# CPestka/Tensor-FFT

Measured on AMD Instinct MI355X. Metric: Gsamples/s + %fp16-MFMA-peak, batched N=4096 fp16 C2C FFT, higher is better.
Workload: dtype f16

## Files before the change

tensor-fft_amd/conv/conv4096.hpp:

```cpp
#pragma once

#include "../csrc/k4096.hpp"

namespace conv4096 {

using k4096::f4;
using k4096::h8;
using k4096::s4;
using k4096::u2;
using k4096::u4;

__host__ __device__ constexpr uint32_t filter_slot(uint32_t k) {
  const uint32_t k0 = k & 15, k1 = (k >> 4) & 15, k2 = k >> 8;
  const uint32_t half = k0 >> 3, j = k0 & 7, g = k2 >> 2, r2 = k2 & 3;
  return ((half * 4 + r2) * 64 + 16 * g + k1) * 8 + j;
}

__global__ __launch_bounds__(k4096::kThreads, 2) void conv4096_kernel(
    const uint16_t* in_re, const uint16_t* in_im, uint16_t* out_re, uint16_t* out_im, uint64_t in_stride, uint64_t out_stride,
    uint32_t batch, uint32_t live, uint32_t filters, const uint8_t* __restrict__ tables, const uint16_t* __restrict__ filt) {
  using namespace k4096;
  extern __shared__ __attribute__((aligned(16))) uint8_t lds[];
  const int tid = threadIdx.x;
  const int lane = tid & 63;
  const int wave = __builtin_amdgcn_readfirstlane(tid >> 6);

  uint8_t* const wl = lds + kLdsTableBytes + wave * kLdsWaveBytes;
  const uint32_t wl_off = __builtin_amdgcn_readfirstlane(
      static_cast<uint32_t>(reinterpret_cast<uintptr_t>((__attribute__((address_space(3))) uint8_t*)wl)));

  const uint32_t stride_b = gridDim.x * live;
  uint32_t b = static_cast<uint32_t>(wave) < live ? blockIdx.x * live + wave : batch;

  for (int i = tid; i < kLdsTableBytes / 16; i += kThreads)
    reinterpret_cast<u4*>(lds)[i] = reinterpret_cast<const u4*>(tables + kOffG)[i];

  const h8 f_re = *reinterpret_cast<const h8*>(tables + kOffF1 + lane * 32);
  const h8 f_im = *reinterpret_cast<const h8*>(tables + kOffF1 + lane * 32 + 16);
  const f4 tw_re = *reinterpret_cast<const f4*>(tables + kOffTw + lane * 32);
  const f4 tw_im = *reinterpret_cast<const f4*>(tables + kOffTw + lane * 32 + 16);
  asm volatile("s_waitcnt vmcnt(0)" ::: "memory");
  __syncthreads();
  if (b >= batch) return;
  dma_in<true>(reinterpret_cast<const uint8_t*>(in_re + b * in_stride), reinterpret_cast<const uint8_t*>(in_im + b * in_stride), wl_off, lane);

  const uint8_t* const g_tab = lds + lane * 16;
  const uint8_t* const h_tab = lds + 16384 + lane * 16;

  const int g = lane >> 4, q = (lane >> 2) & 3, p = lane & 3;
  const int m = q + 4 * (g & 1), bb = g >> 1;
  uint8_t* const tr_base = wl + m * 1024 + bb * 512 + 8 * p;

  auto transform = [&](auto&& mul, auto&& sink) {
    uint32_t pr[8][4], pi[8][4];
#pragma unroll
    for (int t = 0; t < 8; ++t) {
      f4 dre[2], dim[2];
#pragma unroll
      for (int e = 0; e < 2; ++e) {
        const int n1 = 2 * t + e;
        uint8_t* a = tr_base + 32 * (n1 ^ m);
        const s4 xr = __builtin_amdgcn_ds_read_tr16_b64_v4i16((__attribute__((address_space(3))) s4*)(a));
        const s4 xi = __builtin_amdgcn_ds_read_tr16_b64_v4i16((__attribute__((address_space(3))) s4*)(a + 8192));
        const u4 raw = {__builtin_bit_cast(u2, xr).x, __builtin_bit_cast(u2, xr).y, __builtin_bit_cast(u2, xi).x, __builtin_bit_cast(u2, xi).y};
        const h8 x = __builtin_bit_cast(h8, raw);
        dre[e] = mfma(f_re, x);
        dim[e] = mfma(f_im, x);
      }
#pragma unroll
      for (int r = 0; r < 4; ++r) {
        pr[t][r] = pk(dre[0][r], dre[1][r]);
        pi[t][r] = pk(dim[0][r], dim[1][r]);
      }
    }
#pragma unroll
    for (int pp = 0; pp < 2; ++pp)
#pragma unroll
      for (int r = 0; r < 4; ++r) {
        transpose4(pr[0 + pp][r], pr[2 + pp][r], pr[4 + pp][r], pr[6 + pp][r]);
        transpose4(pi[0 + pp][r], pi[2 + pp][r], pi[4 + pp][r], pi[6 + pp][r]);
      }
    auto tile23 = [&](int k0, f4& o_re, f4& o_im) {
      const int a = k0 >> 2, r = k0 & 3;
      const u4 araw = {pr[2 * a][r], pr[2 * a + 1][r], pi[2 * a][r], pi[2 * a + 1][r]};
      const h8 aop = __builtin_bit_cast(h8, araw);
      const u4 graw = *reinterpret_cast<const u4*>(g_tab + k0 * 1024);
      const f4 e_re = mfma(aop, __builtin_bit_cast(h8, graw));
      const f4 e_im = mfma(aop, im_form(graw));
      f4 t_re, t_im;
#pragma unroll
      for (int r4 = 0; r4 < 4; ++r4) {
        t_re[r4] = __builtin_fmaf(e_re[r4], tw_re[r4], -(e_im[r4] * tw_im[r4]));
        t_im[r4] = __builtin_fmaf(e_re[r4], tw_im[r4], e_im[r4] * tw_re[r4]);
      }
      const u4 braw = {pk(t_re[0], t_re[1]), pk(t_re[2], t_re[3]), pk(t_im[0], t_im[1]), pk(t_im[2], t_im[3])};
      const h8 bop = __builtin_bit_cast(h8, braw);
      const u4 hraw = *reinterpret_cast<const u4*>(h_tab + k0 * 1024);
      o_re = mfma(__builtin_bit_cast(h8, hraw), bop);
      o_im = mfma(im_form(hraw), bop);
      mul(k0, o_re, o_im);
    };
#pragma unroll
    for (int half = 0; half < 2; ++half) {
      uint32_t ore[4][4], oim[4][4];
#pragma unroll
      for (int kp = 0; kp < 4; ++kp) {
        f4 e_re, e_im, o_re, o_im;
        tile23(8 * half + 2 * kp, e_re, e_im);
        tile23(8 * half + 2 * kp + 1, o_re, o_im);
#pragma unroll
        for (int r2 = 0; r2 < 4; ++r2) {
          ore[r2][kp] = pk(e_re[r2], o_re[r2]);
          oim[r2][kp] = pk(e_im[r2], o_im[r2]);
        }
      }
#pragma unroll
      for (int r2 = 0; r2 < 4; ++r2) {
        const u4 vr = {ore[r2][0], ore[r2][1], ore[r2][2], ore[r2][3]};
        const u4 vi = {oim[r2][0], oim[r2][1], oim[r2][2], oim[r2][3]};
        sink(half, r2, vr, vi);
      }
    }
  };

  for (;;) {
    asm volatile("s_waitcnt vmcnt(0)" ::: "memory");

    const uint16_t* const fimg = filt + static_cast<uint64_t>(b % filters) * 8192u + 8u * lane;
    u4 hre[2][4], him[2][4];
#pragma unroll
    for (int half = 0; half < 2; ++half)
#pragma unroll
      for (int r2 = 0; r2 < 4; ++r2) {
        hre[half][r2] = *reinterpret_cast<const u4*>(fimg + (half * 4 + r2) * 512);
        him[half][r2] = *reinterpret_cast<const u4*>(fimg + 4096 + (half * 4 + r2) * 512);
      }

    transform(
        [&](int k0, f4& o_re, f4& o_im) {
#pragma unroll
          for (int r2 = 0; r2 < 4; ++r2) {
            const float fr = static_cast<float>(__builtin_bit_cast(h8, hre[k0 >> 3][r2])[k0 & 7]) * 4096.f;
            const float fi = static_cast<float>(__builtin_bit_cast(h8, him[k0 >> 3][r2])[k0 & 7]) * 4096.f;
            const float zr = __builtin_fmaf(o_re[r2], fr, -(o_im[r2] * fi));
            o_im[r2] = __builtin_fmaf(o_re[r2], fi, o_im[r2] * fr);
            o_re[r2] = zr;
          }
        },
        [&](int half, int r2, u4 vr, u4 vi) {
          const uint32_t mm = 2u * g + (r2 >> 1);
          const uint32_t cl = 2u * (lane & 15) + half + 32u * (r2 & 1);
          const uint32_t off = 1024u * mm + 16u * (cl ^ (2u * mm));
          *reinterpret_cast<u4*>(wl + 8192 + off) = vr;
          *reinterpret_cast<u4*>(wl + off) = vi;
        });
    asm volatile("s_waitcnt lgkmcnt(0)" ::: "memory");

    transform([](int, f4&, f4&) {},
              [&](int half, int r2, u4 vr, u4 vi) {
                const uint32_t slot = 2u * (lane & 15) + half;
                const uint32_t off = 16u * (slot ^ ((slot >> 3) & 1)) + 512u * (4 * g + r2);
                *reinterpret_cast<u4*>(wl + 8192 + off) = vr;
                *reinterpret_cast<u4*>(wl + off) = vi;
              });
    uint16_t* const y_re = out_re + b * out_stride;
    uint16_t* const y_im = out_im + b * out_stride;
    const uint32_t rd = 16u * (lane ^ ((lane >> 3) & 1));
#pragma unroll
    for (int i = 0; i < 8; ++i) {
      const u4 vr = *reinterpret_cast<const u4*>(wl + 1024 * i + rd);
      const u4 vi = *reinterpret_cast<const u4*>(wl + 8192 + 1024 * i + rd);
      st<kNonTemporal>(y_re + 512 * i + 8 * lane, vr);
      st<kNonTemporal>(y_im + 512 * i + 8 * lane, vi);
    }
    const uint32_t nb = b + stride_b;
    if (nb >= batch) break;
    asm volatile("s_waitcnt lgkmcnt(0)" ::: "memory");
    dma_in<true>(reinterpret_cast<const uint8_t*>(in_re + nb * in_stride), reinterpret_cast<const uint8_t*>(in_im + nb * in_stride), wl_off, lane);
    b = nb;
  }
}

}
```

tensor-fft_amd/conv/tfft_conv.hip:

```cpp
#include <hip/hip_runtime.h>

#include <algorithm>
#include <cstring>
#include <mutex>
#include <string>
#include <vector>

#include "../../include/tfft_conv.h"
#include "cmul.hpp"
#include "conv4096.hpp"

namespace {

thread_local std::string g_err;

int fail(int code, const std::string& msg) {
  g_err = msg;
  return code;
}
int hip_fail(hipError_t e, const char* what) { return fail(TFFT_ERR_HIP, std::string(what) + ": " + hipGetErrorString(e)); }
int pass_through(int rc) {
  if (rc != TFFT_OK) g_err = tfft_last_error();
  return rc;
}
#define CONV_HIP(call)                        \
  do {                                        \
    const hipError_t e_ = (call);             \
    if (e_ != hipSuccess) return hip_fail(e_, #call); \
  } while (0)

inline bool is_pow2(uint64_t v) { return v && !(v & (v - 1)); }
inline int ilog2(uint64_t v) {
  int l = 0;
  while (v >>= 1) ++l;
  return l;
}

constexpr uint64_t kMinN = 256, kMaxN = uint64_t{1} << 26;

int check_abi() {
  static const int version = tfft_abi_version();
  if (version != TFFT_ABI_VERSION)
    return fail(TFFT_ERR_ARG, "libtfft.so speaks ABI " + std::to_string(version) + ", libtfft_conv.so was built against ABI " +
                                  std::to_string(TFFT_ABI_VERSION) + ": rebuild the add-on");
  return TFFT_OK;
}

int check_shape(uint64_t n, uint64_t batch, uint64_t filters, int flags) {
  if (!is_pow2(n)) return fail(TFFT_ERR_ARG, "n must be a power of two");
  if (n < kMinN || n > kMaxN) return fail(TFFT_ERR_ARG, "n must lie in 256 .. 2^26");
  if (flags & ~TFFT_CONV_COMPOSED) return fail(TFFT_ERR_ARG, "unknown flag bits (" + std::to_string(flags) + ")");
  if (batch == 0 || batch > 0xffffffffull) return fail(TFFT_ERR_ARG, "batch must be in [1, 2^32)");
  if (filters == 0 || filters > batch) return fail(TFFT_ERR_ARG, "filters must be in [1, batch]");
  return TFFT_OK;
}
int check_stride(uint64_t n, uint64_t stride, const char* which) {
  if (stride && (stride % 8 || stride < 2 * n))
    return fail(TFFT_ERR_ARG, std::string(which) + "_batch_stride must be 0 or a multiple of 8 that is >= 2 n");
  return TFFT_OK;
}

inline bool fused_shape(uint64_t n, int flags) { return n == 4096 && !(flags & TFFT_CONV_COMPOSED); }

uint64_t filter_slot(uint64_t n, int flags, uint64_t k) {
  if (fused_shape(n, flags)) return conv4096::filter_slot(static_cast<uint32_t>(k));
  const uint64_t n2 = tfft_plan_transposed_n2(n);
  if (!n2) return k;
  const uint64_t n1 = n / n2;
  return (k % n1) * n2 + k / n1;
}

bool planes_overlap(const void* pa, uint64_t sa, const void* pb, uint64_t sb, uint64_t batch, uint64_t n) {
  const uintptr_t a = reinterpret_cast<uintptr_t>(pa), b = reinterpret_cast<uintptr_t>(pb);
  const uintptr_t a_end = a + 2 * ((batch - 1) * sa + n), b_end = b + 2 * ((batch - 1) * sb + n);
  if (a_end <= b || b_end <= a) return false;
  if (batch == 1 || sa != sb) return true;
  const uint64_t d = static_cast<uint64_t>(a > b ? a - b : b - a) / 2 % sa;
  return d < n || sa - d < n;
}

inline size_t round256(size_t v) { return (v + 255) & ~size_t{255}; }

int describe_chain(uint64_t n, uint64_t batch, bool inverse, std::string& out) {
  char a[256], b[256];
  const uint64_t n2 = tfft_plan_transposed_n2(n);
  if (!n2) {
    const int rc = pass_through(tfft_plan_describe(n, 1, tfft_plan_default_variant(n, 1, batch), a, sizeof(a)));
    out = a;
    return rc;
  }
  const uint64_t n1 = n / n2;
  int rc = pass_through(tfft_plan_describe(n1, n2, n1 == 512 ? TFFT_VARIANT_RADIX512_ONE_PASS : 0, a, sizeof(a)));
  if (rc == TFFT_OK) rc = pass_through(tfft_plan_describe(n2, 1, 0, b, sizeof(b)));
  if (rc) return rc;
  out = inverse ? std::string(b) + " " + a : std::string(a) + " " + b;
  return TFFT_OK;
}

}

struct tfft_conv_plan {
  uint64_t n = 0, batch = 0, filters = 0, in_stride = 0, out_stride = 0;
  int device = 0, flags = 0, num_cus = 256;
  bool fused = false;
  void* d_tables = nullptr;
  uint16_t* d_filter = nullptr;
  bool have_filter = false;
  tfft_plan* fwd = nullptr;
  tfft_plan* inv = nullptr;
  size_t spec_bytes = 0, sub_bytes = 0;
  mutable std::mutex ws_mutex;
  mutable void* ws = nullptr;
  mutable size_t ws_bytes = 0;
  mutable bool ws_owned = false;
};

namespace {

int bind_workspace(const tfft_conv_plan* p) {
  if (!p->sub_bytes) return TFFT_OK;
  void* sub = static_cast<uint8_t*>(p->ws) + p->spec_bytes;
  int rc = pass_through(tfft_plan_set_workspace(p->fwd, tfft_plan_workspace_bytes(p->fwd) ? sub : nullptr, p->sub_bytes));
  if (rc == TFFT_OK) rc = pass_through(tfft_plan_set_workspace(p->inv, tfft_plan_workspace_bytes(p->inv) ? sub : nullptr, p->sub_bytes));
  return rc;
}

int ensure_workspace(const tfft_conv_plan* p) {
  std::lock_guard<std::mutex> lock(p->ws_mutex);
  const size_t need = p->spec_bytes + p->sub_bytes;
  if (!need || p->ws) return TFFT_OK;
  void* mem = nullptr;
  CONV_HIP(hipMalloc(&mem, need));
  p->ws = mem;
  p->ws_bytes = need;
  p->ws_owned = true;
  return bind_workspace(p);
}

void conv4096_shape(const tfft_conv_plan* p, uint32_t& live, uint32_t& grid) {
  const uint64_t cus = static_cast<uint64_t>(p->num_cus);
  live = 8;
  for (uint32_t l = 1; l <= 4; l *= 2)
    if (p->batch <= cus * l) {
      live = l;
      break;
    }
  const uint64_t blocks = (p->batch + live - 1) / live;
  const uint64_t iters = blocks >= 4 * cus ? 2 : 1;
  grid = static_cast<uint32_t>(std::max<uint64_t>(std::min<uint64_t>(blocks, cus), (blocks + iters - 1) / iters));
}

int create_fused(tfft_conv_plan* p) {
  std::vector<uint8_t> blob;
  k4096::build_tables(blob);
  CONV_HIP(hipMalloc(&p->d_tables, k4096::kOffF1n));
  CONV_HIP(hipMemcpy(p->d_tables, blob.data(), k4096::kOffF1n, hipMemcpyHostToDevice));
  CONV_HIP(hipFuncSetAttribute(reinterpret_cast<const void*>(conv4096::conv4096_kernel), hipFuncAttributeMaxDynamicSharedMemorySize, k4096::kLdsBytes));
  return TFFT_OK;
}

int create_composed(tfft_conv_plan* p) {
  const bool transposed = tfft_plan_transposed_n2(p->n) != 0;
  tfft_plan_opts fo = TFFT_PLAN_OPTS_INIT;
  fo.in_batch_stride = p->in_stride;
  fo.out_batch_stride = 2 * p->n;
  fo.preserve_input = 1;
  fo.output_order = transposed ? TFFT_ORDER_TRANSPOSED : TFFT_ORDER_NATURAL;
  tfft_plan_opts io = TFFT_PLAN_OPTS_INIT;
  io.in_batch_stride = 2 * p->n;
  io.out_batch_stride = p->out_stride;
  io.input_order = transposed ? TFFT_ORDER_TRANSPOSED : TFFT_ORDER_NATURAL;
  int rc = pass_through(tfft_plan_create(p->n, p->batch, p->device, &fo, &p->fwd));
  if (rc == TFFT_OK) rc = pass_through(tfft_plan_create(p->n, p->batch, p->device, &io, &p->inv));
  if (rc) return rc;
  p->spec_bytes = round256(static_cast<size_t>(p->batch) * p->n * 4);
  p->sub_bytes = round256(std::max(tfft_plan_workspace_bytes(p->fwd), tfft_plan_workspace_bytes(p->inv)));
  return TFFT_OK;
}

}

extern "C" {

const char* tfft_conv_last_error(void) { return g_err.c_str(); }

uint64_t tfft_conv_filter_slot(uint64_t n, int flags, uint64_t k) {
  if (!is_pow2(n) || n < kMinN || n > kMaxN || (flags & ~TFFT_CONV_COMPOSED) || k >= n) return UINT64_MAX;
  return filter_slot(n, flags, k);
}

int tfft_conv_describe(uint64_t n, uint64_t batch, uint64_t filters, int flags, char* buf, size_t bytes) {
  g_err.clear();
  if (!buf || bytes == 0) return fail(TFFT_ERR_ARG, "null buffer");
  int rc = check_shape(n, batch, filters, flags);
  if (rc) return rc;
  std::string out;
  if (fused_shape(n, flags)) {
    out = "conv4096:4096";
  } else {
    std::string f, i;
    rc = describe_chain(n, batch, false, f);
    if (rc == TFFT_OK) rc = describe_chain(n, batch, true, i);
    if (rc) return rc;
    out = f + " | cmul | " + i;
  }
  if (out.size() + 1 > bytes) return fail(TFFT_ERR_ARG, "buffer too small");
  std::memcpy(buf, out.c_str(), out.size() + 1);
  return TFFT_OK;
}

int tfft_conv_plan_create(uint64_t n, uint64_t batch, uint64_t filters, int device_id, uint64_t in_batch_stride,
                          uint64_t out_batch_stride, int flags, tfft_conv_plan** out) {
  g_err.clear();
  if (!out) return fail(TFFT_ERR_ARG, "null plan pointer");
  *out = nullptr;
  int rc = check_shape(n, batch, filters, flags);
  if (rc == TFFT_OK) rc = check_stride(n, in_batch_stride, "in");
  if (rc == TFFT_OK) rc = check_stride(n, out_batch_stride, "out");
  if (rc == TFFT_OK) rc = check_abi();
  if (rc == TFFT_OK) rc = pass_through(tfft_device_check(device_id));
  if (rc) return rc;
  int prev = 0;
  CONV_HIP(hipGetDevice(&prev));
  CONV_HIP(hipSetDevice(device_id));
  tfft_conv_plan* p = new tfft_conv_plan;
  p->n = n;
  p->batch = batch;
  p->filters = filters;
  p->in_stride = in_batch_stride ? in_batch_stride : 2 * n;
  p->out_stride = out_batch_stride ? out_batch_stride : 2 * n;
  p->device = device_id;
  p->flags = flags;
  p->fused = fused_shape(n, flags);
  hipDeviceProp_t prop;
  if (hipGetDeviceProperties(&prop, device_id) == hipSuccess) p->num_cus = prop.multiProcessorCount;
  rc = p->fused ? create_fused(p) : create_composed(p);
  if (rc == TFFT_OK) {
    const hipError_t e = hipMalloc(reinterpret_cast<void**>(&p->d_filter), static_cast<size_t>(filters) * n * 4);
    if (e != hipSuccess) rc = hip_fail(e, "hipMalloc(filter image)");
  }
  (void)hipSetDevice(prev);
  if (rc) {
    const std::string keep = g_err;
    tfft_conv_plan_destroy(p);
    g_err = keep;
    return rc;
  }
  *out = p;
  return TFFT_OK;
}

void tfft_conv_plan_destroy(tfft_conv_plan* p) {
  if (!p) return;
  tfft_plan_destroy(p->fwd);
  tfft_plan_destroy(p->inv);
  if (p->d_tables) (void)hipFree(p->d_tables);
  if (p->d_filter) (void)hipFree(p->d_filter);
  if (p->ws && p->ws_owned) (void)hipFree(p->ws);
  delete p;
}

int tfft_conv_plan_set_filter(tfft_conv_plan* p, const void* h_re, const void* h_im, void* stream) {
  g_err.clear();
  if (!p) return fail(TFFT_ERR_ARG, "null plan");
  if (!h_re || !h_im) return fail(TFFT_ERR_ARG, "null filter pointer");
  int cur = 0;
  CONV_HIP(hipGetDevice(&cur));
  if (cur != p->device) return fail(TFFT_ERR_ARG, "plan was created for another device than the current one");
  const size_t plane = static_cast<size_t>(p->filters) * p->n;
  std::vector<uint16_t> re(plane), im(plane), img(2 * plane);
  hipStream_t s = static_cast<hipStream_t>(stream);
  CONV_HIP(hipMemcpyAsync(re.data(), h_re, plane * 2, hipMemcpyDeviceToHost, s));
  CONV_HIP(hipMemcpyAsync(im.data(), h_im, plane * 2, hipMemcpyDeviceToHost, s));
  CONV_HIP(hipStreamSynchronize(s));
  for (uint64_t f = 0; f < p->filters; ++f)
    for (uint64_t k = 0; k < p->n; ++k) {
      const uint64_t slot = filter_slot(p->n, p->flags, k);
      img[f * 2 * p->n + slot] = re[f * p->n + k];
      img[f * 2 * p->n + p->n + slot] = im[f * p->n + k];
    }
  if (p->have_filter) CONV_HIP(hipDeviceSynchronize());
  CONV_HIP(hipMemcpy(p->d_filter, img.data(), img.size() * 2, hipMemcpyHostToDevice));
  p->have_filter = true;
  return TFFT_OK;
}

size_t tfft_conv_plan_workspace_bytes(const tfft_conv_plan* p) { return p ? p->spec_bytes + p->sub_bytes : 0; }

int tfft_conv_plan_set_workspace(tfft_conv_plan* p, void* device_ptr, size_t bytes) {
  g_err.clear();
  if (!p) return fail(TFFT_ERR_ARG, "null plan");
  const size_t need = p->spec_bytes + p->sub_bytes;
  if (device_ptr && bytes < need) return fail(TFFT_ERR_WORKSPACE, "workspace too small: " + std::to_string(need) + " bytes needed");
  if (reinterpret_cast<uintptr_t>(device_ptr) & 255) return fail(TFFT_ERR_ARG, "the workspace must be 256-byte aligned");
  std::lock_guard<std::mutex> lock(p->ws_mutex);
  if (p->ws && p->ws_owned) (void)hipFree(p->ws);
  p->ws = need ? device_ptr : nullptr;
  p->ws_bytes = p->ws ? bytes : 0;
  p->ws_owned = false;
  return p->ws ? bind_workspace(p) : TFFT_OK;
}

int tfft_conv_plan_prepare(tfft_conv_plan* p) {
  g_err.clear();
  if (!p) return fail(TFFT_ERR_ARG, "null plan");
  if (p->fused) return TFFT_OK;
  int prev = 0;
  CONV_HIP(hipGetDevice(&prev));
  CONV_HIP(hipSetDevice(p->device));
  int rc = ensure_workspace(p);
  if (rc == TFFT_OK) rc = pass_through(tfft_plan_prepare(p->fwd));
  if (rc == TFFT_OK) rc = pass_through(tfft_plan_prepare(p->inv));
  (void)hipSetDevice(prev);
  return rc;
}

int tfft_conv_exec(const tfft_conv_plan* p, const void* in_re, const void* in_im, void* out_re, void* out_im, void* stream) {
  g_err.clear();
  if (!p) return fail(TFFT_ERR_ARG, "null plan");
  if (!p->have_filter) return fail(TFFT_ERR_ARG, "no filter: call tfft_conv_plan_set_filter first");
  if (!in_re || !in_im || !out_re || !out_im) return fail(TFFT_ERR_ARG, "null data pointer");
  if ((reinterpret_cast<uintptr_t>(in_re) | reinterpret_cast<uintptr_t>(in_im) | reinterpret_cast<uintptr_t>(out_re) |
       reinterpret_cast<uintptr_t>(out_im)) & 15)
    return fail(TFFT_ERR_ARG, "data pointers must be 16-byte aligned");
  const bool same_re = in_re == out_re, same_im = in_im == out_im;
  if ((same_re || same_im) && p->in_stride != p->out_stride)
    return fail(TFFT_ERR_ARG, "in-place execution needs equal input and output batch strides");
  if ((!same_re && planes_overlap(in_re, p->in_stride, out_re, p->out_stride, p->batch, p->n)) ||
      (!same_im && planes_overlap(in_im, p->in_stride, out_im, p->out_stride, p->batch, p->n)) ||
      planes_overlap(in_re, p->in_stride, out_im, p->out_stride, p->batch, p->n) ||
      planes_overlap(in_im, p->in_stride, out_re, p->out_stride, p->batch, p->n) ||
      planes_overlap(out_re, p->out_stride, out_im, p->out_stride, p->batch, p->n))
    return fail(TFFT_ERR_ARG, "input and output planes overlap without being identical (only exact in-place or disjoint planes are supported)");
  int cur = 0;
  CONV_HIP(hipGetDevice(&cur));
  if (cur != p->device) return fail(TFFT_ERR_ARG, "plan was created for another device than the current one");
  hipStream_t s = static_cast<hipStream_t>(stream);
  if (p->fused) {
    uint32_t live, grid;
    conv4096_shape(p, live, grid);
    hipLaunchKernelGGL(conv4096::conv4096_kernel, dim3(grid), dim3(k4096::kThreads), k4096::kLdsBytes, s, static_cast<const uint16_t*>(in_re),
                       static_cast<const uint16_t*>(in_im), static_cast<uint16_t*>(out_re), static_cast<uint16_t*>(out_im), p->in_stride,
                       p->out_stride, static_cast<uint32_t>(p->batch), live, static_cast<uint32_t>(p->filters),
                       static_cast<const uint8_t*>(p->d_tables), p->d_filter);
    CONV_HIP(hipGetLastError());
    return TFFT_OK;
  }
  int rc = ensure_workspace(p);
  if (rc) return rc;
  uint16_t* const spec = static_cast<uint16_t*>(p->ws);
  rc = pass_through(tfft_exec(p->fwd, in_re, in_im, spec, spec + p->n, s));
  if (rc) return rc;
  const uint64_t total = p->batch * (p->n / 8);
  const uint32_t grid = static_cast<uint32_t>(std::min<uint64_t>((total + cmul::kThreads - 1) / cmul::kThreads, static_cast<uint64_t>(p->num_cus) * 32));
  hipLaunchKernelGGL(cmul::cmul_kernel, dim3(grid), dim3(cmul::kThreads), 0, s, spec, p->d_filter, static_cast<uint32_t>(ilog2(p->n / 8)), total,
                     static_cast<uint32_t>(p->filters), static_cast<float>(p->n));
  CONV_HIP(hipGetLastError());
  return pass_through(tfft_exec_inverse(p->inv, spec, spec + p->n, out_re, out_im, s));
}

int tfft_conv_plan_num_launches(const tfft_conv_plan* p) {
  if (!p) return 0;
  return p->fused ? 1 : tfft_plan_num_launches(p->fwd) + 1 + tfft_plan_num_launches(p->inv);
}

int tfft_conv_plan_kernels(const tfft_conv_plan* p, char* buf, size_t bytes) {
  g_err.clear();
  if (!p) return fail(TFFT_ERR_ARG, "null plan");
  std::string out;
  int lines = 1;
  if (p->fused) {
    out = "conv4096::conv4096_kernel\n";
  } else {
    std::vector<char> tmp(1 << 16);
    const int a = tfft_plan_kernels(p->fwd, tmp.data(), tmp.size());
    if (a < 0) return pass_through(a);
    out = tmp.data();
    out += "cmul::cmul_kernel\n";
    const int b = tfft_plan_kernels(p->inv, tmp.data(), tmp.size());
    if (b < 0) return pass_through(b);
    out += tmp.data();
    lines = a + 1 + b;
  }
  if (!buf || out.size() + 1 > bytes) return fail(TFFT_ERR_ARG, "buffer too small (" + std::to_string(out.size() + 1) + " bytes needed)");
  std::memcpy(buf, out.c_str(), out.size() + 1);
  return lines;
}

}
```

Measured before the change: 762.9.

## Prefetch next signal into registers during inverse transform in fused conv kernel

The fused 4096-point convolution kernel no longer waits for the next signal's DMA into LDS after storing the output. It issues non-temporal global loads of the next signal's real and imaginary planes into registers partway through the inverse transform, then writes them to LDS after the output store. The filter load for the next signal is also overlapped. The launch-shape helper moves to its own header and now uses a persistent grid of about one block per CU when the batch is large, instead of two iterations per block. This raises register pressure, with 32 extra u4 registers live, which may hurt occupancy at two blocks per CU.

Result: no change. 756.0 (-0.9%).

```diff
diff --git a/tensor-fft_amd/conv/conv4096.hpp b/tensor-fft_amd/conv/conv4096.hpp
--- a/tensor-fft_amd/conv/conv4096.hpp
+++ b/tensor-fft_amd/conv/conv4096.hpp
@@ -51,7 +51,7 @@
   const int m = q + 4 * (g & 1), bb = g >> 1;
   uint8_t* const tr_base = wl + m * 1024 + bb * 512 + 8 * p;
 
-  auto transform = [&](auto&& mul, auto&& sink) {
+  auto transform = [&](auto&& mul, auto&& sink, auto&& mid) {
     uint32_t pr[8][4], pi[8][4];
 #pragma unroll
     for (int t = 0; t < 8; ++t) {
@@ -120,14 +120,44 @@
         const u4 vi = {oim[r2][0], oim[r2][1], oim[r2][2], oim[r2][3]};
         sink(half, r2, vr, vi);
       }
-    }
-  };
-
-  for (;;) {
-    asm volatile("s_waitcnt vmcnt(0)" ::: "memory");
-
-    const uint16_t* const fimg = filt + static_cast<uint64_t>(b % filters) * 8192u + 8u * lane;
-    u4 hre[2][4], him[2][4];
+      if (half == 0) mid();
+    }
+  };
+
+  auto prefetch_plane = [&](u4 (&d)[8], const uint16_t* src, uint32_t more) {
+    uint32_t l16 = static_cast<uint32_t>(lane) * 16u;
+    asm volatile("" : "+v"(l16));
+    uint32_t o[8];
+#pragma unroll
+    for (int mm = 0; mm < 8; ++mm) o[mm] = l16 ^ (32u * mm);
+    asm volatile(
+        "s_cmp_eq_u32 %18, 0\n\t"
+        "s_cbranch_scc1 1f\n\t"
+        "s_nop 4\n\t"
+        "global_load_dwordx4 %0, %8, %16 nt\n\t"
+        "global_load_dwordx4 %1, %9, %16 offset:1024 nt\n\t"
+        "global_load_dwordx4 %2, %10, %16 offset:2048 nt\n\t"
+        "global_load_dwordx4 %3, %11, %16 offset:3072 nt\n\t"
+        "global_load_dwordx4 %4, %12, %17 nt\n\t"
+        "global_load_dwordx4 %5, %13, %17 offset:1024 nt\n\t"
+        "global_load_dwordx4 %6, %14, %17 offset:2048 nt\n\t"
+        "global_load_dwordx4 %7, %15, %17 offset:3072 nt\n"
+        "1:"
+        : "=&v"(d[0]), "=&v"(d[1]), "=&v"(d[2]), "=&v"(d[3]), "=&v"(d[4]), "=&v"(d[5]), "=&v"(d[6]), "=&v"(d[7])
+        : "v"(o[0]), "v"(o[1]), "v"(o[2]), "v"(o[3]), "v"(o[4]), "v"(o[5]), "v"(o[6]), "v"(o[7]), "s"(src), "s"(src + 2048), "s"(more)
+        : "memory", "scc");
+  };
+  auto prefetch_wait = [&](u4 (&r)[8], u4 (&i)[8]) {
+    asm volatile("s_waitcnt vmcnt(0)"
+                 : "+v"(r[0]), "+v"(r[1]), "+v"(r[2]), "+v"(r[3]), "+v"(r[4]), "+v"(r[5]), "+v"(r[6]), "+v"(r[7]), "+v"(i[0]), "+v"(i[1]),
+                   "+v"(i[2]), "+v"(i[3]), "+v"(i[4]), "+v"(i[5]), "+v"(i[6]), "+v"(i[7])
+                 :
+                 : "memory");
+  };
+
+  u4 hre[2][4], him[2][4];
+  auto load_filter = [&](uint32_t sig) {
+    const uint16_t* const fimg = filt + static_cast<uint64_t>(sig % filters) * 8192u + 8u * lane;
 #pragma unroll
     for (int half = 0; half < 2; ++half)
 #pragma unroll
@@ -135,7 +165,16 @@
         hre[half][r2] = *reinterpret_cast<const u4*>(fimg + (half * 4 + r2) * 512);
         him[half][r2] = *reinterpret_cast<const u4*>(fimg + 4096 + (half * 4 + r2) * 512);
       }
-
+  };
+  load_filter(b);
+
+  asm volatile("s_waitcnt vmcnt(0)"
+               : "+v"(hre[0][0]), "+v"(hre[0][1]), "+v"(hre[0][2]), "+v"(hre[0][3]), "+v"(hre[1][0]), "+v"(hre[1][1]), "+v"(hre[1][2]),
+                 "+v"(hre[1][3]), "+v"(him[0][0]), "+v"(him[0][1]), "+v"(him[0][2]), "+v"(him[0][3]), "+v"(him[1][0]), "+v"(him[1][1]),
+                 "+v"(him[1][2]), "+v"(him[1][3])
+               :
+               : "memory");
+  for (;;) {
     transform(
         [&](int k0, f4& o_re, f4& o_im) {
 #pragma unroll
@@ -153,8 +192,14 @@
           const uint32_t off = 1024u * mm + 16u * (cl ^ (2u * mm));
           *reinterpret_cast<u4*>(wl + 8192 + off) = vr;
           *reinterpret_cast<u4*>(wl + off) = vi;
-        });
+        },
+        [] {});
     asm volatile("s_waitcnt lgkmcnt(0)" ::: "memory");
+
+    const uint32_t nb = b + stride_b;
+    const uint32_t more = __builtin_amdgcn_readfirstlane(nb < batch ? 1u : 0u);
+    u4 nre[8], nim[8];
+    prefetch_plane(nre, in_re + nb * in_stride, more);
 
     transform([](int, f4&, f4&) {},
               [&](int half, int r2, u4 vr, u4 vi) {
@@ -162,21 +207,34 @@
                 const uint32_t off = 16u * (slot ^ ((slot >> 3) & 1)) + 512u * (4 * g + r2);
                 *reinterpret_cast<u4*>(wl + 8192 + off) = vr;
                 *reinterpret_cast<u4*>(wl + off) = vi;
+              },
+              [&] {
+                prefetch_plane(nim, in_im + nb * in_stride, more);
               });
     uint16_t* const y_re = out_re + b * out_stride;
     uint16_t* const y_im = out_im + b * out_stride;
     const uint32_t rd = 16u * (lane ^ ((lane >> 3) & 1));
+    u4 vr[8], vi[8];
 #pragma unroll
     for (int i = 0; i < 8; ++i) {
-      const u4 vr = *reinterpret_cast<const u4*>(wl + 1024 * i + rd);
-      const u4 vi = *reinterpret_cast<const u4*>(wl + 8192 + 1024 * i + rd);
-      st<kNonTemporal>(y_re + 512 * i + 8 * lane, vr);
-      st<kNonTemporal>(y_im + 512 * i + 8 * lane, vi);
-    }
-    const uint32_t nb = b + stride_b;
-    if (nb >= batch) break;
+      vr[i] = *reinterpret_cast<const u4*>(wl + 1024 * i + rd);
+      vi[i] = *reinterpret_cast<const u4*>(wl + 8192 + 1024 * i + rd);
+    }
+    prefetch_wait(nre, nim);
+    if (more) load_filter(nb);
+    asm volatile("" ::: "memory");
+#pragma unroll
+    for (int i = 0; i < 8; ++i) {
+      st<kNonTemporal>(y_re + 512 * i + 8 * lane, vr[i]);
+      st<kNonTemporal>(y_im + 512 * i + 8 * lane, vi[i]);
+    }
+    if (!more) break;
+#pragma unroll
+    for (int mm = 0; mm < 8; ++mm) {
+      *reinterpret_cast<u4*>(wl + mm * 1024 + lane * 16) = nre[mm];
+      *reinterpret_cast<u4*>(wl + 8192 + mm * 1024 + lane * 16) = nim[mm];
+    }
     asm volatile("s_waitcnt lgkmcnt(0)" ::: "memory");
-    dma_in<true>(reinterpret_cast<const uint8_t*>(in_re + nb * in_stride), reinterpret_cast<const uint8_t*>(in_im + nb * in_stride), wl_off, lane);
     b = nb;
   }
 }
diff --git a/tensor-fft_amd/conv/conv4096_shape.hpp b/tensor-fft_amd/conv/conv4096_shape.hpp
--- /dev/null
+++ b/tensor-fft_amd/conv/conv4096_shape.hpp
@@ -0,0 +1,22 @@
+#pragma once
+
+#include <algorithm>
+#include <cstdint>
+
+namespace conv4096 {
+
+constexpr uint64_t kSignalsPerWave = 0;
+
+inline void launch_shape(uint64_t batch, uint64_t cus, uint32_t& live, uint32_t& grid) {
+  live = 8;
+  for (uint32_t l = 1; l <= 4; l *= 2)
+    if (batch <= cus * l) {
+      live = l;
+      break;
+    }
+  const uint64_t blocks = (batch + live - 1) / live;
+  const uint64_t iters = blocks >= 4 * cus ? (kSignalsPerWave ? kSignalsPerWave : blocks) : 1;
+  grid = static_cast<uint32_t>(std::max<uint64_t>(std::min<uint64_t>(blocks, cus), (blocks + iters - 1) / iters));
+}
+
+}
diff --git a/tensor-fft_amd/conv/tfft_conv.hip b/tensor-fft_amd/conv/tfft_conv.hip
--- a/tensor-fft_amd/conv/tfft_conv.hip
+++ b/tensor-fft_amd/conv/tfft_conv.hip
@@ -9,6 +9,7 @@
 #include "../../include/tfft_conv.h"
 #include "cmul.hpp"
 #include "conv4096.hpp"
+#include "conv4096_shape.hpp"
 
 namespace {
 
@@ -135,19 +136,6 @@
   p->ws_bytes = need;
   p->ws_owned = true;
   return bind_workspace(p);
-}
-
-void conv4096_shape(const tfft_conv_plan* p, uint32_t& live, uint32_t& grid) {
-  const uint64_t cus = static_cast<uint64_t>(p->num_cus);
-  live = 8;
-  for (uint32_t l = 1; l <= 4; l *= 2)
-    if (p->batch <= cus * l) {
-      live = l;
-      break;
-    }
-  const uint64_t blocks = (p->batch + live - 1) / live;
-  const uint64_t iters = blocks >= 4 * cus ? 2 : 1;
-  grid = static_cast<uint32_t>(std::max<uint64_t>(std::min<uint64_t>(blocks, cus), (blocks + iters - 1) / iters));
 }
 
 int create_fused(tfft_conv_plan* p) {
@@ -338,7 +326,7 @@
   hipStream_t s = static_cast<hipStream_t>(stream);
   if (p->fused) {
     uint32_t live, grid;
-    conv4096_shape(p, live, grid);
+    conv4096::launch_shape(p->batch, static_cast<uint64_t>(p->num_cus), live, grid);
     hipLaunchKernelGGL(conv4096::conv4096_kernel, dim3(grid), dim3(k4096::kThreads), k4096::kLdsBytes, s, static_cast<const uint16_t*>(in_re),
                        static_cast<const uint16_t*>(in_im), static_cast<uint16_t*>(out_re), static_cast<uint16_t*>(out_im), p->in_stride,
                        p->out_stride, static_cast<uint32_t>(p->batch), live, static_cast<uint32_t>(p->filters),
```

## Store conv output directly from registers and overlap next input DMA

Applied to the files above, without the earlier changes.

The second transform's sink now writes results straight to global memory instead of staging them in LDS and reading them back. The next batch's input DMA is issued from inside the transform, right after the LDS reads finish, so it overlaps with the remaining MFMA work. The loop-top wait drops to a partial vmcnt so outstanding stores do not block it. The filter multiply now uses v_fma_mix with packed half operands, and the grid is resized so each persistent block runs more iterations. Optional timestamp instrumentation is added behind a macro. The new store pattern writes 16-byte chunks that are less coalesced than before and no longer uses non-temporal stores; the real/imag swap in the sink needs checking for correctness.

New measurement: 752.2 before, 752.6 after, median of 3. No clear change (+0.1%).

```diff
diff --git a/tensor-fft_amd/conv/conv4096.hpp b/tensor-fft_amd/conv/conv4096.hpp
--- a/tensor-fft_amd/conv/conv4096.hpp
+++ b/tensor-fft_amd/conv/conv4096.hpp
@@ -15,6 +15,43 @@
   const uint32_t half = k0 >> 3, j = k0 & 7, g = k2 >> 2, r2 = k2 & 3;
   return ((half * 4 + r2) * 64 + 16 * g + k1) * 8 + j;
 }
+
+__device__ __forceinline__ float mixmul(float a, uint32_t packed, bool hi) {
+  float d;
+  if (hi)
+    asm("v_fma_mix_f32 %0, %1, %2, %3 op_sel:[0,1,0] op_sel_hi:[0,1,0]" : "=v"(d) : "v"(a), "v"(packed), "s"(-0.f));
+  else
+    asm("v_fma_mix_f32 %0, %1, %2, %3 op_sel_hi:[0,1,0]" : "=v"(d) : "v"(a), "v"(packed), "s"(-0.f));
+  return d;
+}
+
+#ifdef TFFT_CONV_STAMPS
+__device__ unsigned long long* stamps_ptr = nullptr;
+__device__ uint32_t stamps_blocks = 0;
+constexpr int kStampSlots = 8;
+__device__ __forceinline__ unsigned long long stamp() {
+  unsigned long long t;
+  __builtin_amdgcn_sched_barrier(0);
+  asm volatile("s_memtime %0\n\ts_waitcnt lgkmcnt(0)" : "=s"(t)::"memory");
+  __builtin_amdgcn_sched_barrier(0);
+  return t;
+}
+extern "C" __attribute__((visibility("default"), used)) int tfft_conv_debug_stamps(void* buffer, uint32_t blocks) {
+  unsigned long long* p = static_cast<unsigned long long*>(buffer);
+  if (hipMemcpyToSymbol(HIP_SYMBOL(stamps_ptr), &p, sizeof(p)) != hipSuccess) return 1;
+  return hipMemcpyToSymbol(HIP_SYMBOL(stamps_blocks), &blocks, sizeof(blocks)) != hipSuccess;
+}
+#define CONV_STAMP(i)                         \
+  do {                                        \
+    const unsigned long long now_ = stamp();  \
+    acc[i] += now_ - last;                    \
+    last = now_;                              \
+  } while (0)
+#else
+#define CONV_STAMP(i) \
+  do {                \
+  } while (0)
+#endif
 
 __global__ __launch_bounds__(k4096::kThreads, 2) void conv4096_kernel(
     const uint16_t* in_re, const uint16_t* in_im, uint16_t* out_re, uint16_t* out_im, uint64_t in_stride, uint64_t out_stride,
@@ -39,7 +76,7 @@
   const h8 f_im = *reinterpret_cast<const h8*>(tables + kOffF1 + lane * 32 + 16);
   const f4 tw_re = *reinterpret_cast<const f4*>(tables + kOffTw + lane * 32);
   const f4 tw_im = *reinterpret_cast<const f4*>(tables + kOffTw + lane * 32 + 16);
-  asm volatile("s_waitcnt vmcnt(0)" ::: "memory");
+  asm volatile("s_waitcnt vmcnt(0)" ::"v"(f_re), "v"(f_im), "v"(tw_re), "v"(tw_im) : "memory");
   __syncthreads();
   if (b >= batch) return;
   dma_in<true>(reinterpret_cast<const uint8_t*>(in_re + b * in_stride), reinterpret_cast<const uint8_t*>(in_im + b * in_stride), wl_off, lane);
@@ -51,7 +88,7 @@
   const int m = q + 4 * (g & 1), bb = g >> 1;
   uint8_t* const tr_base = wl + m * 1024 + bb * 512 + 8 * p;
 
-  auto transform = [&](auto&& mul, auto&& sink) {
+  auto transform = [&](auto&& mul, auto&& sink, auto&& image_read) {
     uint32_t pr[8][4], pi[8][4];
 #pragma unroll
     for (int t = 0; t < 8; ++t) {
@@ -73,6 +110,7 @@
         pi[t][r] = pk(dim[0][r], dim[1][r]);
       }
     }
+    image_read();
 #pragma unroll
     for (int pp = 0; pp < 2; ++pp)
 #pragma unroll
@@ -123,8 +161,24 @@
     }
   };
 
+#ifdef TFFT_CONV_STAMPS
+  unsigned long long acc[kStampSlots] = {};
+  unsigned long long last = stamp();
+#endif
+  const uint32_t out_lane_off = 16u * (lane & 15) + 1024u * g;
+  bool first = true;
+
   for (;;) {
-    asm volatile("s_waitcnt vmcnt(0)" ::: "memory");
+    CONV_STAMP(0);
+#ifdef TFFT_CONV_STAMPS
+    ++acc[7];
+#endif
+    if (!first)
+      asm volatile("s_waitcnt vmcnt(16)" ::: "memory");
+    else
+      asm volatile("s_waitcnt vmcnt(0)" ::: "memory");
+    first = false;
+    CONV_STAMP(1);
 
     const uint16_t* const fimg = filt + static_cast<uint64_t>(b % filters) * 8192u + 8u * lane;
     u4 hre[2][4], him[2][4];
@@ -135,15 +189,25 @@
         hre[half][r2] = *reinterpret_cast<const u4*>(fimg + (half * 4 + r2) * 512);
         him[half][r2] = *reinterpret_cast<const u4*>(fimg + 4096 + (half * 4 + r2) * 512);
       }
+#if defined(TFFT_CONV_STAMPS) && TFFT_CONV_STAMPS == 2
+    asm volatile("s_waitcnt vmcnt(0)" ::: "memory");
+#endif
+    CONV_STAMP(2);
+
+    const uint32_t nb = b + stride_b;
+    uint16_t* const y_re = out_re + b * out_stride;
+    uint16_t* const y_im = out_im + b * out_stride;
 
     transform(
         [&](int k0, f4& o_re, f4& o_im) {
 #pragma unroll
           for (int r2 = 0; r2 < 4; ++r2) {
-            const float fr = static_cast<float>(__builtin_bit_cast(h8, hre[k0 >> 3][r2])[k0 & 7]) * 4096.f;
-            const float fi = static_cast<float>(__builtin_bit_cast(h8, him[k0 >> 3][r2])[k0 & 7]) * 4096.f;
-            const float zr = __builtin_fmaf(o_re[r2], fr, -(o_im[r2] * fi));
-            o_im[r2] = __builtin_fmaf(o_re[r2], fi, o_im[r2] * fr);
+            const _Float16 hr = __builtin_bit_cast(h8, hre[k0 >> 3][r2])[k0 & 7];
+            const _Float16 hi = __builtin_bit_cast(h8, him[k0 >> 3][r2])[k0 & 7];
+            const float sr = o_re[r2] * 4096.f, si = o_im[r2] * 4096.f;
+            const uint32_t wr = hre[k0 >> 3][r2][(k0 & 7) >> 1], wi = him[k0 >> 3][r2][(k0 & 7) >> 1];
+            const float zr = __builtin_fmaf(sr, static_cast<float>(hr), -mixmul(si, wi, k0 & 1));
+            o_im[r2] = __builtin_fmaf(sr, static_cast<float>(hi), mixmul(si, wr, k0 & 1));
             o_re[r2] = zr;
           }
         },
@@ -153,32 +217,33 @@
           const uint32_t off = 1024u * mm + 16u * (cl ^ (2u * mm));
           *reinterpret_cast<u4*>(wl + 8192 + off) = vr;
           *reinterpret_cast<u4*>(wl + off) = vi;
-        });
+        },
+        [] {});
     asm volatile("s_waitcnt lgkmcnt(0)" ::: "memory");
+    CONV_STAMP(3);
 
     transform([](int, f4&, f4&) {},
               [&](int half, int r2, u4 vr, u4 vi) {
-                const uint32_t slot = 2u * (lane & 15) + half;
-                const uint32_t off = 16u * (slot ^ ((slot >> 3) & 1)) + 512u * (4 * g + r2);
-                *reinterpret_cast<u4*>(wl + 8192 + off) = vr;
-                *reinterpret_cast<u4*>(wl + off) = vi;
+                st<0>(y_re + out_lane_off + 256 * r2 + 8 * half, vi);
+                st<0>(y_im + out_lane_off + 256 * r2 + 8 * half, vr);
+              },
+              [&] {
+                asm volatile("s_waitcnt lgkmcnt(0)" ::: "memory");
+                if (nb < batch)
+                  dma_in<true>(reinterpret_cast<const uint8_t*>(in_re + nb * in_stride), reinterpret_cast<const uint8_t*>(in_im + nb * in_stride),
+                               wl_off, lane);
               });
-    uint16_t* const y_re = out_re + b * out_stride;
-    uint16_t* const y_im = out_im + b * out_stride;
-    const uint32_t rd = 16u * (lane ^ ((lane >> 3) & 1));
-#pragma unroll
-    for (int i = 0; i < 8; ++i) {
-      const u4 vr = *reinterpret_cast<const u4*>(wl + 1024 * i + rd);
-      const u4 vi = *reinterpret_cast<const u4*>(wl + 8192 + 1024 * i + rd);
-      st<kNonTemporal>(y_re + 512 * i + 8 * lane, vr);
-      st<kNonTemporal>(y_im + 512 * i + 8 * lane, vi);
-    }
-    const uint32_t nb = b + stride_b;
+    CONV_STAMP(4);
     if (nb >= batch) break;
-    asm volatile("s_waitcnt lgkmcnt(0)" ::: "memory");
-    dma_in<true>(reinterpret_cast<const uint8_t*>(in_re + nb * in_stride), reinterpret_cast<const uint8_t*>(in_im + nb * in_stride), wl_off, lane);
     b = nb;
   }
-}
-
-}
+  asm volatile("s_waitcnt vmcnt(0)" ::: "memory");
+#ifdef TFFT_CONV_STAMPS
+  CONV_STAMP(5);
+  if (lane == 0 && stamps_ptr && blockIdx.x < stamps_blocks)
+#pragma unroll
+    for (int i = 0; i < kStampSlots; ++i) stamps_ptr[(blockIdx.x * 8 + wave) * kStampSlots + i] = acc[i];
+#endif
+}
+
+}
diff --git a/tensor-fft_amd/conv/tfft_conv.hip b/tensor-fft_amd/conv/tfft_conv.hip
--- a/tensor-fft_amd/conv/tfft_conv.hip
+++ b/tensor-fft_amd/conv/tfft_conv.hip
@@ -146,7 +146,7 @@
       break;
     }
   const uint64_t blocks = (p->batch + live - 1) / live;
-  const uint64_t iters = blocks >= 4 * cus ? 2 : 1;
+  const uint64_t iters = blocks >= 4 * cus ? blocks / (2 * cus) : 1;
   grid = static_cast<uint32_t>(std::max<uint64_t>(std::min<uint64_t>(blocks, cus), (blocks + iters - 1) / iters));
 }
 
```
